# HKPolyU-UAV/bluerov2

Measured on AMD Instinct MI355X. Metric: NMPC RTI solves/s (N=20, 12 states / 4 inputs), batch 4096 per GPU, higher is better.
Workload: dtype f64; 1 GPU; BASELINE.json configs[1]: batch=4096 independent BlueROV2 NMPC instances per GPU, N=20, Ts=0.05 s, circle reference window advancing one row per step, per-instance x0 noise (seed 1), nominal parameters, default options (qp_early_exit=1: exact equality-constrained shortcut when no bound is active); batch_per_gpu=4096, N=20, parallelism=single GPU

## Files before the change

bluerov2_amd/csrc/qp/fused.hpp:

```cpp
#pragma once

namespace brov {

constexpr int kFusedMaxN = 23;
template <int W, bool GRID, bool DF>
__device__ __forceinline__ bool rti_fused_step(const DevParams& P, int b, int lane, bool listed, size_t yoff) {
    extern __shared__ __attribute__((aligned(16))) double smem[];
    const int N = P.N;
    double* ba_s = smem;
    double* bv_s = ba_s + (size_t)N * kBaStage;
    double* kt_s = bv_s + (size_t)N * NX;
    double* kff_s = kt_s + (size_t)N * kKtStage;
    double* vh_s = kff_s + (size_t)N * 4;
    double* dx_s = vh_s + (size_t)N * 4;
    double* q_s = dx_s + (size_t)(N + 1) * NX;
    double* r_s = q_s + (size_t)(N + 1) * NX;
    double* const_s = r_s + (size_t)N * 4;
    if (lane == 0) { const_s[0] = 0.0; const_s[1] = 1.0; }
    LaneCst lc;
    if constexpr (W == 1) lc = load_lane_cst(P.cst, lane);
    double part = 0.0;
    bool nanp = false;
    lin_phase<W == 1, GRID>(P, b, 0, N, lane, ba_s, bv_s, kt_s, q_s, r_s, part, nanp, true, yoff);
    __syncthreads();
    if (P.dump_lin) copy_out_linearisation(P, b, 0, N, lane, ba_s, bv_s);
    std::conditional_t<GRID, InstGrid, Inst> I;
    setup_inst(P, I, b, lane, W == 1 ? &lc : nullptr, yoff);
    const bool listed_u = __builtin_amdgcn_readfirstlane((int)listed) != 0;
    I.ckpt = (N >= 8 && P.partial_refactor && listed_u) ? (N + 3) >> 2 : 0;
    I.lds_ba = (const lds_f64*)ba_s;
    I.lds_bv = (const lds_f64*)bv_s;
    I.lds_kt = (lds_f64*)kt_s;
    I.lds_q = (const lds_f64*)q_s;
    I.lds_r = (const lds_f64*)r_s;
    I.kff = kff_s;
    I.vhat = vh_s;
    I.dxb = dx_s;
    I.lds_kff = (lds_f64*)kff_s;
    I.lds_vhat = (lds_f64*)vh_s;
    I.lds_dxb = (lds_f64*)dx_s;
    I.lds_zero = (lds_f64*)const_s;
    I.lds_tr = (lds_f64*)const_s + 2;
    {
        const int rg = I.rg, cl = I.cl;
        const int zero = (int)(const_s - ba_s), one = zero + 1, kt0 = (int)(kt_s - ba_s);
        for (int r = 0; r < 3; r++) I.ba_off[r] = cl >= 3 ? (rg + 4 * r) * kBaStride + cl - 3 : ((r == 0 && rg == cl) ? one : zero);
        I.ba_str = cl >= 3 ? kBaStage : 0;
        for (int r = 0; r < 4; r++) {
            const int c = rg + 4 * r;
            I.bat_off[r] = cl >= NX ? zero : (c >= 3 ? cl * kBaStride + c - 3 : (c == cl ? one : zero));
        }
        I.bat_str = cl >= NX ? 0 : kBaStage;
        I.bat_str0 = (cl < NX && rg == 3) ? kBaStage : 0;
        for (int r = 0; r < 3; r++) I.kt_off[r] = cl < 4 ? kt0 + (rg + 4 * r) * 4 + cl : zero;
        I.kt_str = cl < 4 ? kKtStage : 0;
    }
    qp_body<W, std::conditional_t<GRID, InstGrid, Inst>, DF>(P, I, b, part, nanp);
    return I.ran_loop;
}
__device__ __forceinline__ void plant_step_wave(const DevParams& P, int b, int lane, int tk) {
    double x[NX], u[NU], k[NX], xs[NX], acc[NX];
    double* x0 = P.x0_rw + (size_t)b * NX;
#pragma unroll
    for (int j = 0; j < NX; j++) x[j] = x0[j];
#pragma unroll
    for (int j = 0; j < NU; j++) u[j] = P.res[b].u0[j];
    const ModelPar m = make_par(P.plant_pp + (size_t)b * NP);
    Wrench w = make_wrench(u);
    if (P.plant_rp) { w.k3 = P.plant_rp[(size_t)b * P.plant_rp_stride]; w.k4 = P.plant_rp[(size_t)b * P.plant_rp_stride + 1]; }
    const double h = P.plant_dt / P.plant_substeps;
    StagePoint sp;
    for (int s = 0; s < P.plant_substeps; s++) {
        model_f(x, w, m, NoWorldWrench{}, k, sp);
#pragma unroll
        for (int j = 0; j < NX; j++) { acc[j] = x[j] + (h / 6.0) * k[j]; xs[j] = x[j] + 0.5 * h * k[j]; }
        model_f(xs, w, m, NoWorldWrench{}, k, sp);
#pragma unroll
        for (int j = 0; j < NX; j++) { acc[j] += (h / 3.0) * k[j]; xs[j] = x[j] + 0.5 * h * k[j]; }
        model_f(xs, w, m, NoWorldWrench{}, k, sp);
#pragma unroll
        for (int j = 0; j < NX; j++) { acc[j] += (h / 3.0) * k[j]; xs[j] = x[j] + h * k[j]; }
        model_f(xs, w, m, NoWorldWrench{}, k, sp);
#pragma unroll
        for (int j = 0; j < NX; j++) x[j] = acc[j] + (h / 6.0) * k[j];
    }
    if (lane == 0) {
#pragma unroll
        for (int j = 0; j < NX; j++) x0[j] = x[j];
        if (P.plant_xlog) {
#pragma unroll
            for (int j = 0; j < NX; j++) P.plant_xlog[((size_t)tk * P.B + b) * NX + j] = x[j];
        }
        if (P.plant_ulog) {
#pragma unroll
            for (int j = 0; j < NU; j++) P.plant_ulog[((size_t)tk * P.B + b) * NU + j] = u[j];
        }
    }
}

template <int W, bool GRID = false, bool DF = false, bool MULTI = false>
__device__ __forceinline__ void rti_fused_body(const DevParams& P) {
    const int b = __builtin_amdgcn_readfirstlane(sched_map(P, blockIdx.x));
    const int lane = threadIdx.x;
    bool listed = sched_listed(P, b);
    if (blockIdx.x == 0) sched_zero_next(P, lane);
    DBG_STAMP(0);
    if constexpr (!MULTI) {
        (void)rti_fused_step<W, GRID, DF>(P, b, lane, listed, 0);
    } else {
#pragma clang loop unroll(disable)
        for (int tk = 0; tk < P.ticks; tk++) {
            int bq = b, lq = lane;
            asm volatile("s_mov_b32 %0, %0" : "+s"(bq));
            asm volatile("v_mov_b32 %0, %0" : "+v"(lq));
            listed = rti_fused_step<W, GRID, DF>(P, bq, lq, listed, (size_t)tk * (size_t)P.tick_yref);
            if (P.tick_status && lq == 0) P.tick_status[(size_t)tk * P.B + bq] = P.res[bq].status;
            __syncthreads();
            wave_fence();
            if (P.plant_pp) {
                plant_step_wave(P, bq, lq, tk);
                __syncthreads();
                wave_fence();
            }
        }
    }
}

}
```

bluerov2_amd/csrc/qp/qp_body.hpp:

```cpp
#pragma once

namespace brov {

#define DBG_STAMP(slot) do { if (P.dbg && lane == 0) {                                                                          \
        P.dbg[(size_t)b * 8 + (slot)] = __builtin_readcyclecounter();                                                           \
        if ((slot) == 0) P.dbg[(size_t)P.B * 8 + (size_t)b * 8 + 7] = __builtin_amdgcn_s_memrealtime();                        \
        if ((slot) == 0) P.dbg[(size_t)P.B * 8 + (size_t)b * 8 + 5] = ((unsigned long long)__builtin_amdgcn_s_getreg(63508) << 32) | __builtin_amdgcn_s_getreg(63492); \
        if ((slot) == 6) P.dbg[(size_t)P.B * 8 + (size_t)b * 8 + 6] = __builtin_amdgcn_s_memrealtime(); } } while (0)
#ifdef BROV_DBG_IPM
#define IPM_T(k) do { const unsigned long long t_ = __builtin_readcyclecounter(); ipm_t[k] += t_ - ipm_last; ipm_last = t_; } while (0)
#else
#define IPM_T(k) do { } while (0)
#endif

#ifdef BROV_DBG_LIN
#define LIN_T(k) do { __builtin_amdgcn_sched_barrier(0); lin_t[k] = __builtin_readcyclecounter(); __builtin_amdgcn_sched_barrier(0); } while (0)
#else
#define LIN_T(k) do { } while (0)
#endif

template <int LDS, class IT = Inst, bool DF = false, bool LONGV = false>
__device__ __forceinline__ void qp_body(const DevParams& P, IT& I, int b, double lin_part, bool lin_nan, Win* W = nullptr,
                                        bool pre_ok = true, bool pre_illc = false) {
    constexpr bool EL = (LDS == 1 || LDS == 2);
    const double* __restrict__ cst = P.cst;
    const int lane = I.lane, N = I.NT, nv = I.nv;
    DBG_STAMP(1);
    const int rg = I.rg;

    double* x_it = P.x + (size_t)b * (N + 1) * 12;
    double* u_it = P.u + (size_t)b * N * 4;
    double* pi_it = P.pi + (size_t)b * N * 12;
    double* lam_it = P.lam + (size_t)b * N * 8;
    double* V = I.ipm + (size_t)IPM_V * nv;
    double* TL = I.ipm + (size_t)IPM_TL * nv;
    double* TU = I.ipm + (size_t)IPM_TU * nv;
    double* LL = I.ipm + (size_t)IPM_LL * nv;
    double* LU = I.ipm + (size_t)IPM_LU * nv;
    double* GAM = I.ipm + (size_t)IPM_GAM * nv;
    double* RT = I.ipm + (size_t)IPM_RT * nv;
    double* DVA = I.ipm + (size_t)IPM_DVA * nv;
    double* ACT = I.ipm + (size_t)IPM_ACT * nv;
    const double* GRAD = EL ? (const double*)I.kff : (const double*)DVA;
    auto rd_vhat = [&](int j) -> double { if constexpr (EL) return I.lds_vhat[j]; else return I.vhat[j]; };
    auto wr_vhat = [&](int j, double v) { if constexpr (EL) I.lds_vhat[j] = v; else I.vhat[j] = v; };
    auto rd_dxb = [&](int j) -> double { if constexpr (EL) return I.lds_dxb[j]; else return I.dxb[j]; };
    auto rd_grad = [&](int j) -> double { if constexpr (EL) return I.lds_kff[j]; else return GRAD[j]; };

    double x0v[3], xiv[3];
    {
        const double* x0 = P.x0 + (size_t)b * 12;
#pragma unroll
        for (int r = 0; r < 3; r++) { x0v[r] = x0[rg + 4 * r]; xiv[r] = I.x[rg + 4 * r]; }
    }

    double ureg[2] = {0.0, 0.0};
    if constexpr (EL) {
#pragma unroll
        for (int t = 0; t < 2; t++)
            if (lane + 64 * t < nv) ureg[t] = I.u[lane + 64 * t];
    }
    int status = 0, iters = 0;
    double mu = 0.0, rho = 0.0;
    bool early = false, polished = false, use_vhat = false;
    int sched_p = -1;
    bool ok = pre_ok;
    constexpr bool PART = EL || LDS >= 3;
    bool illc0 = pre_illc;
    bool split0 = false;
    if constexpr (EL) split0 = I.ckpt > 0;
    if constexpr (EL) { if (split0) {
        BwdState S;
        wave_fence();
        bwd_init<true, LDS>(I, S);
#pragma clang loop unroll(disable)
        for (int ph = 0; ph < 2; ph++) {
            if (ph == 1) {
                if (I.ckpt == 0) break;
                double* ck = I.Kt;
#pragma unroll
                for (int r = 0; r < 3; r++) { ck[r * 64 + lane] = S.P[r]; ck[192 + r * 64 + lane] = S.pv[r]; }
            }
            bwd_chunk<true, LDS, false, true>(I, S, ph == 0 ? N : I.ckpt, ph == 0 ? I.ckpt : 0);
        }
        ok = S.ok;
        illc0 = S.illc;
    } }
    if constexpr (LDS < 3) { if (!split0) ok = riccati_backward<true, LDS, false, true>(I, &illc0); }
    d4 d0;
    double kkt = 0.0;
    {
#pragma unroll
        for (int r = 0; r < 3; r++) {
            d0[r] = x0v[r] - xiv[r];
            kkt_upd(kkt, d0[r]);
        }
        d0[3] = 0.0;
        double part = lin_part;
        bool nanp = lin_nan;
        if (kkt != kkt) nanp = true;
        kkt = wave_max(fmax(part, (kkt != kkt) ? 0.0 : kkt));
        if (__ballot(nanp) != 0ull) kkt = __builtin_nan("");
    }
    constexpr bool ROB = LDS != 2;
    bool robust = false, robust_ok = false;
    if constexpr (ROB) {
        robust_ok = kkt <= P.robust_kkt_max || P.robust_pivot == 3;
        if ((__ballot(illc0) != 0ull && P.robust_pivot && robust_ok) || P.robust_pivot == 2) {
            robust = true;
            I.ckpt = 0;
            ok = sw_backward<true, LDS, true, true>(I, W);
        }
    }
    DBG_STAMP(2);
    const double lbc = EL ? cst[32 + (lane & 3)] : 0.0, ubc = EL ? cst[36 + (lane & 3)] : 0.0;
    if (__ballot(!ok) != 0ull) {
        status = BROV_STATUS_QP_FAILURE;
    } else {
        sw_forward<LDS>(I, W, d0, cst);
        DBG_STAMP(3);
        bool feas = true;
        if constexpr (LDS >= 3) {
            feas = W->feas;
        } else if constexpr (EL) {
#pragma unroll
            for (int t = 0; t < 2; t++) {
                const int j = lane + 64 * t;
                if (j < nv) {
                    const double vj = rd_vhat(j), lb = lbc - ureg[t], ub = ubc - ureg[t];
                    if (!(vj >= lb && vj <= ub)) feas = false;
                }
            }
        } else {
            for (int j = lane; j < nv; j += 64) {
                const int m = j & 3;
                const double vj = rd_vhat(j), lb = cst[32 + m] - I.u[j], ub = cst[36 + m] - I.u[j];
                if (!(vj >= lb && vj <= ub)) feas = false;
            }
        }
        const bool allfeas = (__ballot(!feas) == 0ull);
        if (allfeas && P.early_exit) {
            early = true;
        } else {
#ifdef BROV_DBG_IPM
            unsigned long long ipm_t[8] = {0, 0, 0, 0, 0, 0, 0, 0}, ipm_last = __builtin_readcyclecounter();
#endif
            constexpr bool CACHE = (LDS >= 3) && !LONGV;
            constexpr int kIpmT = EL ? 2 : ((LDS == 0 || LONGV) ? 16 : 8);
            using Vec = IpmVec<EL ? 1 : (CACHE ? 2 : 0), kIpmT>;
            Vec vV{{}, V}, vTL{{}, TL}, vTU{{}, TU}, vLL{{}, LL}, vLU{{}, LU}, vDVA{{}, DVA},
                vDLL{{}, GAM}, vDLU{{}, RT},
                vACT{{}, ACT};
#define IPM_FOR(t, j) _Pragma("unroll") for (int t = 0; t < kIpmT; t++) if (const unsigned j = (unsigned)lane + 64u * t; j < (unsigned)nv)
#define IPM_PRE(arr, expr)                                                                     \
            double arr[CACHE ? kIpmT : 1];                                                         \
            if constexpr (CACHE) {                                                                 \
                _Pragma("unroll") for (int t = 0; t < kIpmT; t++) {                                \
                    const unsigned j = ((unsigned)lane + 64u * t < (unsigned)nv) ? (unsigned)lane + 64u * t : 0u; \
                    arr[t] = (expr);                                                               \
                }                                                                                  \
            }
            auto set_act = [&](int t, int j, double v) __attribute__((always_inline)) { if constexpr (CACHE) ACT[j] = v; else vACT.set(t, j, v); };
#define GROUP_LANE int lane_g_ = I.lane; asm volatile("v_mov_b32 %0, %0" : "+v"(lane_g_)); const int lane = lane_g_
            const int mI = lane & 3;
            double lbI = cst[32 + mI], ubI = cst[36 + mI], wuI = cst[12 + mI];
            asm volatile("" : "+v"(lbI), "+v"(ubI), "+v"(wuI));
            const double rdI = P.Ts * wuI;
            auto rd_el = [&](unsigned j) __attribute__((always_inline)) -> double {
                if constexpr (LDS == 0) return I.wst ? I.wst[(size_t)(j >> 2) * 16 + 12 + mI] : rdI;
                else if constexpr (IT::kGrid) return I.wst[(size_t)(j >> 2) * 16 + 12 + mI];
                else return rdI;
            };
            {
                GROUP_LANE;
// ... 261 lines not shown
                    amax = wave_min(amax);
                    {
                        const double a = amax < 1.0 ? amax : 1.0;
                        alpha = (IPM_FTB * amax >= 1.0) ? 1.0 : a * ((1.0 - a) * IPM_FTBLO + a * IPM_FTB);
                    }
                    IPM_FOR(t, j) {
                        const double dv = (CACHE ? vh[CACHE ? t : 0] : rd_vhat(j)) - vV.get(t, j);
                        const double vj = vV.get(t, j) + alpha * dv;
                        const double tl = vTL.get(t, j) + alpha * dv, tu = vTU.get(t, j) - alpha * dv;
                        double dll, dlu;
                        if constexpr (CACHE) {
                            const double l0 = vLL.get(t, j), u0_ = vLU.get(t, j), t0_ = vTL.get(t, j), t1_ = vTU.get(t, j), dva = vDVA.get(t, j);
                            const double dlla = -l0 - l0 / t0_ * dva, dlua = -u0_ + u0_ / t1_ * dva;
                            dll = (smu - dlla * dva) / t0_ - l0 - l0 / t0_ * dv;
                            dlu = (smu + dlua * dva) / t1_ - u0_ + u0_ / t1_ * dv;
                        } else {
                            dll = vDLL.get(t, j); dlu = vDLU.get(t, j);
                        }
                        const double ll = vLL.get(t, j) + alpha * dll, lu = vLU.get(t, j) + alpha * dlu;
                        vV.set(t, j, vj); vTL.set(t, j, tl); vTU.set(t, j, tu); vLL.set(t, j, ll); vLU.set(t, j, lu);
                        if (!(vj == vj)) bad = true;
                        s2 += ll * tl + lu * tu;
                        const double rde = rd_el(j), al = ll / rde, au = lu / rde;
                        unres = fmax(unres, fmax(fmin(tl, al), fmin(tu, au)));
                        set_act(t, j, al > tl ? -1.0 : (au > tu ? 1.0 : 0.0));
                    }
                    vV.flush(lane, nv); vTL.flush(lane, nv); vTU.flush(lane, nv); vLL.flush(lane, nv); vLU.flush(lane, nv);
                    }
                if (__ballot(bad) != 0ull) { status = BROV_STATUS_NAN; break; }
                rho *= (1.0 - alpha);
                mu = wave_sum(s2) * inv2nv;
                IPM_T(1);
                unres = wave_max(unres);
                if (unres <= P.tol_mu && rho <= P.tol_stat) converged = true;
                if (converged || (mu <= POL_MU_GATE * mu_gate && alpha >= POL_ALPHA_GATE)) { round_k = 0; round_cap = POL_LOOP; nchg_prev = nv + 1; }
            }
            if (converged && status == BROV_STATUS_MAXITER) status = BROV_STATUS_SUCCESS;
#ifdef BROV_DBG_IPM
            if (P.dbg && lane == 0) {
                ipm_t[6] = iters;
                for (int k = 0; k < 7; k++) P.dbg[(size_t)P.B * 8 + (size_t)b * 8 + k] = ipm_t[k];
            }
#endif
            use_vhat = polished || !ipm_on;
            if (!polished) {
                if (ipm_on) {
                    if constexpr (EL) { IPM_FOR(t, j) wr_vhat(j, vV.get(t, j)); }
                } else if (status == BROV_STATUS_MAXITER) {
                    GROUP_LANE;
                    IPM_PRE(up, I.u[j]);
                    IPM_PRE(vh, I.vhat[j]);
                    IPM_FOR(t, j) {
                        const double uj = EL ? ureg[t & 1] : (CACHE ? up[CACHE ? t : 0] : I.u[j]);
                        double vj = CACHE ? vh[CACHE ? t : 0] : rd_vhat(j);
                        vj = fmin(fmax(vj, lbI - uj), ubI - uj);
                        if constexpr (EL) wr_vhat(j, vj); else I.vhat[j] = vj;
                    }
                }
            }
#undef IPM_FOR
#undef IPM_PRE
#undef GROUP_LANE
        }
    }

    bool emitted = false;
    auto emit_record = [&](double cost_lane, double u0_lane, bool have_u0) __attribute__((always_inline)) {
        const double cs = wave_sum(cost_lane);
        if (lane == 0) {
            brov_result* r = P.res + b;
            r->cost = cs;
            r->kkt = kkt;
            r->status = status;
            r->qp_iter = early ? 0 : iters;
        }
        double u0r = u0_lane;
        if (!have_u0 && lane < 4) {
            u0r = P.res[b].u0[lane];
            u0r = (u0r == u0r) ? u0r : 0.0;
            u0r = fmin(fmax(u0r, cst[32 + lane]), cst[36 + lane]);
            P.res[b].u0[lane] = u0r;
        }
        const double a0 = readlane_f64(u0r, 0), a1 = readlane_f64(u0r, 1), a2 = readlane_f64(u0r, 2), a3 = readlane_f64(u0r, 3);
        const double s0 = (lane == 0 || lane == 1) ? -a0 : a0;
        const double s1 = (lane == 0 || lane == 2) ? a1 : -a1;
        const double s3 = (lane == 0 || lane == 3) ? a3 : -a3;
        const double th = ((lane < 4) ? (s0 + s1) + s3 : -a2) / kRotor;
        if (lane < 6) P.res[b].thrust[lane] = th;
        if (P.mail) {
            brov_result* m = P.mail + b;
            if (lane < 4) m->u0[lane] = u0r;
            if (lane < 6) m->thrust[lane] = th;
            if (lane == 0) { m->cost = cs; m->kkt = kkt; m->status = status; m->qp_iter = early ? 0 : iters; }
            if (P.mail_flag) {
                __threadfence_system();
                if (lane == 0) __hip_atomic_store(P.mail_flag + b, P.mail_seq, __ATOMIC_RELEASE, __HIP_MEMORY_SCOPE_SYSTEM);
            }
        }
        emitted = true;
    };

    constexpr int UX = EL ? 5 : 4, UU = EL ? 2 : 4;
    const double* vfin = (early || EL || use_vhat) ? I.vhat : V;
    const int nxe = (N + 1) * 12;
    double cost = 0.0;
    bool wrote_u0 = false;
    double u0v = 0.0;
    if (status == BROV_STATUS_SUCCESS || status == BROV_STATUS_MAXITER) {
        if (!early && !polished) {
            sw_rollout<LDS>(I, W, d0, vfin);
        }
        DBG_STAMP(4);
        if constexpr (LDS >= 3) {
            if (W->nan) {
                status = BROV_STATUS_NAN;
            } else {
                win_adjoint_commit<LDS == 4>(P, I, *W, b, vfin, early, cost, u0v, P.mail != nullptr && P.mail_early != 0,
                                             [&](double cost_lane, double u0_lane) __attribute__((always_inline)) { emit_record(cost_lane, u0_lane, true); });
                wrote_u0 = true;
            }
            DBG_STAMP(5);
        } else {
        double xpre[UX], ypre[UX], urpre[UU];
        double wxpre[LDS == 1 ? UX : 1], wupre[LDS == 1 ? UU : 1];
        if constexpr (EL) {
#pragma unroll
            for (int t = 0; t < UX; t++) {
                const int j = lane + 64 * t;
                const int jj = j < nxe ? j : 0;
                const int i = div12(jj), c = jj - i * 12;
                xpre[t] = x_it[jj];
                ypre[t] = I.yref[(size_t)i * 16 + c];
                if constexpr (LDS == 1) wxpre[t] = cst[(i == N) ? 16 + c : c];
            }
#pragma unroll
            for (int t = 0; t < UU; t++) {
                const int j = lane + 64 * t;
                const int jj = j < nv ? j : 0;
                urpre[t] = I.yref[(size_t)(jj >> 2) * 16 + 12 + (jj & 3)];
                if constexpr (LDS == 1) wupre[t] = cst[12 + (jj & 3)];
            }
        }
        auto copy_pi = [&]() __attribute__((always_inline)) {
            double pv5[5];
#pragma unroll
            for (int t = 0; t < 5; t++) pv5[t] = I.lds_kt[lane + 64 * t < N * 12 ? lane + 64 * t : 0];
#pragma unroll
            for (int t = 0; t < 5; t++) asm volatile("" : "+v"(pv5[t]));
#pragma unroll
            for (int t = 0; t < 5; t++)
                if (lane + 64 * t < N * 12) pi_it[lane + 64 * t] = pv5[t];
        };
        const bool late = DF && EL && early && P.mail != nullptr;
        if (!(EL && polished) && !late) sw_adjoint<true, LDS>(I, W, vfin, DVA, pi_it);
        DBG_STAMP(5);
        bool nanv = false;
        double vvp[EL ? UU : 1], djp[EL ? UX : 1];
        if constexpr (EL) {
#pragma unroll
            for (int t = 0; t < UU; t++) vvp[t] = rd_vhat(lane + 64 * t < nv ? lane + 64 * t : 0);
#pragma unroll
            for (int t = 0; t < UX; t++) djp[t] = rd_dxb(lane + 64 * t < nxe ? lane + 64 * t : 0);
#pragma unroll
            for (int t = 0; t < UU; t++) nanv = nanv || !(vvp[t] == vvp[t]);
#pragma unroll
            for (int t = 0; t < UX; t++) nanv = nanv || !(djp[t] == djp[t]);
        } else {
            for (int j = lane; j < nv; j += 64) {
                const double vj = vfin[j];
                if (!(vj == vj)) nanv = true;
            }
            for (int j = lane; j < nxe; j += 64) {
                const double dj = rd_dxb(j);
                if (!(dj == dj)) nanv = true;
            }
        }
        if (__ballot(nanv) != 0ull) {
            status = BROV_STATUS_NAN;
        } else {
            for (int j0 = lane; j0 < nv; j0 += 64 * UU) {
                double uo[UU], vv[UU], gg[UU], ur[UU];
#pragma unroll
                for (int t = 0; t < UU; t++) {
                    const int j = j0 + 64 * t;
                    const bool in = j < nv;
                    const int jj = in ? j : 0;
                    uo[t] = (EL && j0 == lane && t < 2) ? ureg[t] : u_it[jj];
                    vv[t] = EL ? ((j0 == lane) ? vvp[EL ? t : 0] : rd_vhat(jj)) : vfin[jj];
                    gg[t] = early ? 0.0 : rd_grad(jj);
                    ur[t] = (EL && j0 == lane) ? urpre[t] : I.yref[(size_t)(jj >> 2) * 16 + 12 + (jj & 3)];
                }
#pragma unroll
                for (int t = 0; t < UU; t++) {
                    const int j = j0 + 64 * t;
                    if (j < nv) {
                        const int i = j >> 2, m = j & 3;
                        lam_it[i * 8 + m] = gg[t] > 0 ? gg[t] : 0.0;
                        lam_it[i * 8 + 4 + m] = gg[t] < 0 ? -gg[t] : 0.0;
                        const double un = uo[t] + vv[t];
                        u_it[j] = un;
                        if (j < 4) { P.res[b].u0[j] = un; u0v = un; }
                        const double e = un - ur[t];
                        const double wgt = (LDS == 1 && j0 == lane) ? wupre[LDS == 1 ? t : 0] : cst[12 + m];
                        const double sw = (IT::kGrid || (LDS == 0 && I.wst)) ? I.wst[(size_t)i * 16 + 12 + m] : P.Ts * wgt;
                        cost += 0.5 * sw * e * e;
                    }
                }
            }
            wrote_u0 = true;
            if constexpr (EL) {
                if (!late) copy_pi();
            }
            for (int j0 = lane; j0 < nxe; j0 += 64 * UX) {
                double xo[UX], dj[UX], yr[UX];
#pragma unroll
                for (int t = 0; t < UX; t++) {
                    const int j = j0 + 64 * t;
                    const int jj = j < nxe ? j : 0;
                    const int i = div12(jj), c = jj - i * 12;
                    xo[t] = (EL && j0 == lane) ? xpre[t] : x_it[jj];
                    dj[t] = (EL && j0 == lane) ? djp[EL ? t : 0] : rd_dxb(jj);
                    yr[t] = (EL && j0 == lane) ? ypre[t] : I.yref[(size_t)i * 16 + c];
                }
#pragma unroll
                for (int t = 0; t < UX; t++) {
                    const int j = j0 + 64 * t;
                    if (j < nxe) {
                        const int i = div12(j), c = j - i * 12;
                        const double xn = xo[t] + dj[t];
                        x_it[j] = xn;
                        const double e = xn - yr[t];
                        const double wgt = (LDS == 1 && j0 == lane) ? wxpre[LDS == 1 ? t : 0] : cst[(i == N) ? 16 + c : c];
                        const double sw = (IT::kGrid || (LDS == 0 && I.wst)) ? I.wst[(size_t)i * 16 + c] : ((i == N) ? wgt : P.Ts * wgt);
                        cost += 0.5 * sw * e * e;
                    }
                }
            }
        }
        if constexpr (DF && EL) {
            if (late && status == BROV_STATUS_SUCCESS) {
                emit_record(cost, u0v, wrote_u0);
                sw_adjoint<true, LDS>(I, W, vfin, DVA, pi_it);
                copy_pi();
            } else if (late) {
            }
        }
        }
    }
    if (status != BROV_STATUS_SUCCESS && status != BROV_STATUS_MAXITER) {
        const double* x0 = P.x0 + (size_t)b * 12;
        const double xl = x0[lane < 12 ? lane : 0];
        const bool restart = P.on_failure == BROV_ON_FAILURE_RESTART && __ballot(!(fabs(xl) < 1e300)) == 0ull;
        for (int j = lane; j < nv; j += 64) {
            const int i = j >> 2, m = j & 3;
            const double e = u_it[j] - I.yref[(size_t)i * 16 + 12 + m];
            cost += 0.5 * ((IT::kGrid || (LDS == 0 && I.wst)) ? I.wst[(size_t)i * 16 + 12 + m] : P.Ts * cst[12 + m]) * e * e;
            if (restart) { u_it[j] = 0.0; lam_it[i * 8 + m] = 0.0; lam_it[i * 8 + 4 + m] = 0.0; }
        }
        for (int j = lane; j < nxe; j += 64) {
            const int i = j / 12, c = j - i * 12;
            const double e = x_it[j] - I.yref[(size_t)i * 16 + c];
            cost += 0.5 * ((IT::kGrid || (LDS == 0 && I.wst)) ? I.wst[(size_t)i * 16 + c] : ((i == N) ? cst[16 + c] : P.Ts * cst[c])) * e * e;
            if (restart) { x_it[j] = x0[c]; if (i < N) pi_it[j] = 0.0; }
        }
    }
    if (!emitted) emit_record(cost, u0v, wrote_u0);
#ifdef BROV_SCHED_TICKET_LATE
    if (sched_p == -2) sched_p = sched_ticket(P, b);
#endif
    sched_note(P, b, sched_p);
    I.ran_loop = !early;
    DBG_STAMP(6);
}


struct LaneCst { double Wr[4], Wer[3], lbm, ubm, Wq, Weq, Wuq; };
__device__ __forceinline__ LaneCst load_lane_cst(const double* __restrict__ cst, int lane) {
    const int rg = lane >> 4;
    LaneCst c;
#pragma unroll
    for (int r = 0; r < 4; r++) c.Wr[r] = cst[rg + 4 * r];
#pragma unroll
    for (int r = 0; r < 3; r++) c.Wer[r] = cst[16 + rg + 4 * r];
    c.lbm = cst[32 + rg];
    c.ubm = cst[36 + rg];
    const int cq = (lane >> 2) < NX ? (lane >> 2) : NX - 1;
    c.Wq = cst[cq];
    c.Weq = cst[16 + cq];
    c.Wuq = cst[12 + ((lane >> 2) & 3)];
    return c;
}
__device__ __forceinline__ void setup_inst(const DevParams& P, Inst& I, int b, int lane, const LaneCst* pre = nullptr, size_t yoff = 0) {
    const int N = P.N, nv = 4 * N;
    const double* __restrict__ cst = P.cst;
    I.lane = lane; I.rg = lane >> 4; I.cl = lane & 15; I.N = N; I.nv = nv;
    I.i0 = 0; I.NT = N; I.ckpt = 0;
    I.x = P.x + (size_t)b * (N + 1) * 12;
    I.u = P.u + (size_t)b * N * 4;
    I.yref = P.yref + yoff + (size_t)b * P.yref_stride;
    I.BA = P.BA + (size_t)b * N * 192;
    I.bvec = P.bvec + (size_t)b * N * 12;
    I.Ks = P.Ks + (size_t)b * N * 64;
    I.Kt = P.Kt + (size_t)b * N * 192;
    I.Mt = P.Mt + (size_t)b * N * 64;
    I.Pb = P.Pb + (size_t)b * N * 12;
    I.kff = P.kff + (size_t)b * N * 4;
    I.vhat = P.vhat + (size_t)b * N * 4;
    I.ipm = P.ipm + (size_t)b * IPM_NARR * nv;
    I.dxb = P.dxb + (size_t)b * (N + 1) * 12;
    I.Ts = P.Ts;
    I.wst = P.wst;
    I.lds_ba = nullptr;
    I.lds_bv = nullptr;
    I.lds_kt = nullptr;
    I.lds_q = nullptr;
    I.lds_r = nullptr;
    I.lds_kff = nullptr;
    I.lds_vhat = nullptr;
    I.lds_dxb = nullptr;
    I.lds_zero = nullptr;
    I.lds_tr = nullptr;
    const LaneCst c = pre ? *pre : load_lane_cst(cst, lane);
#pragma unroll
    for (int r = 0; r < 4; r++) I.Wr[r] = c.Wr[r];
#pragma unroll
    for (int r = 0; r < 3; r++) I.Wer[r] = c.Wer[r];
    I.lbm = c.lbm;
    I.ubm = c.ubm;
    I.Wq = c.Wq; I.Weq = c.Weq; I.Wuq = c.Wuq;
}

}
```

bluerov2_amd/csrc/qp/sweeps.hpp:

```cpp
#pragma once

namespace brov {

template <int LDS> constexpr int kLdsDist = LDS == 2 ? 1 : 2;

struct BwdIn {
    d4 ba;
    d4 bv;
    double xv[3], yv[3];
    double rtv, gm;
    double ks, mt;
};

struct Ba1Off { int off[3], str; };
template <bool FACTOR, int LDS, bool STEP0 = false, class IT = Inst>
__device__ __forceinline__ BwdIn load_bwd(const IT& I, int i, const double* gam, const double* rt, const Ba1Off* b1 = nullptr) {
    BwdIn s;
    s.ba = get_ba<LDS>(I, i);
    const int ig = I.i0 + i;
    if constexpr (FACTOR && LDS != 0) {
        if (b1) {
            const lds_f64* t = I.lds_ba + lmul(i, b1->str);
            s.bv = d4{t[b1->off[0]], t[b1->off[1]], t[b1->off[2]], 0.0};
        } else {
// ... 551 lines not shown
        const bool rowx = k < NX;
        const double e0 = (q == 0 && k == 0) ? 1.0 : 0.0, e1 = (q == 0 && k == 1) ? 1.0 : 0.0, e2 = (q == 0 && k == 2) ? 1.0 : 0.0;
        lds_f64* xpark = rowx ? I.lds_dxb + NX + k : I.lds_tr + (I.lane & 15);
        const int xstr = rowx ? NX : 0;
        const int ka = rowx ? k : NX - 1, c0 = 4 * q - 3;
        const int oa = ka * kBaStride + (c0 > 0 ? c0 : 0), oa3 = ka * kBaStride + c0 + 3, ob = ka;
        const lds_f64* zr0 = q < 3 ? I.lds_dxb + 4 * q : I.lds_vhat;
        const int zstr = q < 3 ? NX : 4;
        double z0 = zr0[0], z1 = zr0[1], z2 = zr0[2], z3 = zr0[3];
        pipelined<kLdsDist<LDS>, RollV>(N, [&](int kk) { return load_roll_v(I, oa, oa3, ob, kk); }, [&](int i, const RollV& in) {
            const double a0 = q == 0 ? e0 : in.a[0], a1 = q == 0 ? e1 : in.a[1], a2 = q == 0 ? e2 : in.a[2];
            double pa = a0 * z0;
            pa = fma(a1, z1, pa); pa = fma(a2, z2, pa); pa = fma(in.a[3], z3, pa);
            const double xn = quad_sum(pa) + in.bk;
            xpark[lmul(i, xstr)] = rowx ? xn : 0.0;
            const lds_f64* zr = zr0 + lmul(i + 1 < N ? i + 1 : i, zstr);
            z0 = zr[0]; z1 = zr[1]; z2 = zr[2]; z3 = zr[3];
        });
        const lds_f64* xl = I.lds_dxb + N * NX + rg;
        xx = d4{xl[0], xl[4], xl[8], 0.0};
    } else {
        pipelined<3, RollIn>(N, [&](int k) { return load_roll<LDS>(I, k, varr); }, [&](int i, const RollIn& in) {
            d4 z = {xx[0], xx[1], xx[2], in.v};
            xx = tn<4>(in.bat, z, in.bb);
            xx[3] = 0.0;
            store_vec12(I.dxb + (size_t)(i + 1) * 12, xx, rg, cl);
        });
    }
}
template <int LDS>
__device__ void rollout(const Inst& I, const d4& d0, const double* varr) {
    wave_fence();
    d4 xx = d0;
    roll_chunk<LDS>(I, xx, varr);
    wave_fence();
}

struct AdjIn { d4 ba; double dx[3], xn[3], yn[3]; double v, u, ur; };
template <int LDS>
__device__ __forceinline__ AdjIn load_adj(const Inst& I, int i, const double* varr) {
    AdjIn s;
    s.ba = get_ba<LDS>(I, i);
    const double* dxn = I.dxb + (size_t)(i + 1) * 12;
    if constexpr (LDS) s.v = I.lds_vhat[i * 4 + I.rg]; else s.v = varr[i * 4 + I.rg];
    if constexpr (LDS) {
        const lds_f64* dxl = I.lds_dxb + (i + 1) * 12;
#pragma unroll
        for (int r = 0; r < 3; r++) { s.dx[r] = dxl[I.rg + 4 * r]; s.xn[r] = I.lds_q[(i + 1) * 12 + I.rg + 4 * r]; s.yn[r] = 0.0; }
        s.u = I.lds_r[i * 4 + I.rg];
        s.ur = 0.0;
    } else {
        const double* xn = I.x + (size_t)(i + 1) * 12;
        const double* yn = I.yref + (size_t)(i + 1) * 16;
#pragma unroll
        for (int r = 0; r < 3; r++) { s.dx[r] = dxn[I.rg + 4 * r]; s.xn[r] = xn[I.rg + 4 * r]; s.yn[r] = yn[I.rg + 4 * r]; }
        s.u = I.u[i * 4 + I.rg];
        s.ur = I.yref[(size_t)i * 16 + 12 + I.rg];
    }
    return s;
}
struct AdjV { double m[4], dxc, qc, vm, rm, wq, wr; };
template <class IT = Inst>
__device__ __forceinline__ AdjV load_adj_v(const IT& I, int om, int ox, int ou, int i) {
    AdjV s;
    const lds_f64* col = I.lds_ba + i * kBaStage + om;
#pragma unroll
    for (int t = 0; t < 4; t++) s.m[t] = col[t * kBaStride];
    s.dxc = I.lds_dxb[(i + 1) * NX + ox];
    s.qc = I.lds_q[(i + 1) * NX + ox];
    s.vm = I.lds_vhat[i * 4 + ou];
    s.rm = I.lds_r[i * 4 + ou];
    s.wq = 0.0; s.wr = 0.0;
    if constexpr (IT::kGrid) {
        s.wq = I.wst[(size_t)(I.i0 + i + 1) * 16 + ox];
        s.wr = I.wst[(size_t)(I.i0 + i) * 16 + 12 + ou];
    }
    return s;
}
template <bool COMMIT, int LDS, class IT = Inst>
__device__ __forceinline__ void adj_chunk(const IT& I, d4& atpi, const double* varr, double* garr, double* pi_out) {
    const int rg = I.rg, cl = I.cl, N = I.N;
    if constexpr (LDS) {
        const int c = I.lane >> 2, q = I.lane & 3;
        const bool rowx = c < NX, colx = q < 3;
        const int q3 = colx ? q : 2;
        const double e0 = (colx && 4 * q == c) ? 1.0 : 0.0, e1 = (colx && 4 * q + 1 == c) ? 1.0 : 0.0, e2 = (colx && 4 * q + 2 == c) ? 1.0 : 0.0,
                     e3 = (colx && 4 * q + 3 == c) ? 1.0 : 0.0;
        const bool ecol = c < 3;
        const int om = (4 * q3) * kBaStride + (c >= 3 ? c - 3 : 0), ox = rowx ? c : NX - 1, ou = c & 3;
        store_vec12_lds(I.lds_tr, atpi, rg, cl);
        double gq = I.lds_tr[rowx ? c : 0];
        lds_f64* ppark = rowx ? I.lds_kt + c : I.lds_tr + (I.lane & 15);
        const int pstr = rowx ? NX : 0;
        lds_f64* gpark = rowx ? I.lds_tr + (I.lane & 15) : I.lds_kff + (c - NX);
        const int gstr = rowx ? 0 : 4;
        const double rd = I.Ts * I.Wuq;
        lds_f64* pp = ppark + lmul(N - 1, pstr);
        lds_f64* gp = gpark + lmul(N - 1, gstr);
        pipelined<kLdsDist<LDS>, AdjV>(N, [&](int kk) { return load_adj_v(I, om, ox, ou, N - 1 - kk); }, [&](int kk, const AdjV& in) {
            const int i = N - 1 - kk;
            const double qd = IT::kGrid ? in.wq : ((I.i0 + i + 1 == I.NT) ? I.Weq : I.Ts * I.Wq);
            const double pic = fma(qd, in.dxc, in.qc + gq);
            *pp = pic; pp -= pstr;
            const lds_f64* pr = I.lds_kt + i * NX + 4 * q3;
            const double p0 = pr[0], p1 = pr[1], p2 = pr[2], p3 = pr[3];
            __builtin_amdgcn_sched_barrier(0);
            const double m0 = ecol ? e0 : in.m[0], m1 = ecol ? e1 : in.m[1], m2 = ecol ? e2 : in.m[2], m3 = ecol ? e3 : in.m[3];
            double acc = m0 * p0;
            acc = fma(m1, p1, acc); acc = fma(m2, p2, acc); acc = fma(m3, p3, acc);
            acc = colx ? acc : 0.0;
            const double G = quad_sum(acc);
            *gp = fma(IT::kGrid ? in.wr : rd, in.vm, in.rm + G); gp -= gstr;
            gq = G;
        });
        lds_f64* tpark = rowx ? I.lds_tr + c : I.lds_tr + 16;
        *tpark = gq;
        const lds_f64* tl = I.lds_tr + rg;
        atpi = d4{tl[0], tl[4], tl[8], 0.0};
        return;
    }
    const d4 z4 = {0, 0, 0, 0};
    auto stage = [&](int i, const AdjIn& in) __attribute__((always_inline)) {
        d4 pi;
        double wq[3], wr;
        if (I.wst) {
            const double* ws = I.wst + (size_t)(i + 1) * 16 + rg;
            wq[0] = ws[0]; wq[1] = ws[4]; wq[2] = ws[8];
            wr = I.wst[(size_t)i * 16 + 12 + rg];
        } else {
#pragma unroll
            for (int r = 0; r < 3; r++) wq[r] = (I.i0 + i + 1 == I.NT) ? I.Wer[r] : I.Ts * I.Wr[r];
            wr = I.Ts * I.Wr[3];
        }
#pragma unroll
        for (int r = 0; r < 3; r++) pi[r] = wq[r] * (in.dx[r] + in.xn[r] - in.yn[r]) + atpi[r];
        pi[3] = 0.0;
        if (COMMIT) store_vec12(pi_out + (size_t)i * 12, pi, rg, cl);
        d4 G = tn<3>(in.ba, pi, z4);
        const double rd = wr;
        if (cl == 0) garr[i * 4 + rg] = rd * in.v + rd * (in.u - in.ur) + G[3];
        atpi = G;
    };
    pipelined<3, AdjIn>(N, [&](int k) { return load_adj<LDS>(I, N - 1 - k, varr); },
                        [&](int k, const AdjIn& in) { stage(N - 1 - k, in); });
}
template <bool COMMIT, int LDS, class IT = Inst>
__device__ void adjoint(const IT& I, const double* varr, double* garr, double* pi_out) {
    wave_fence();
    d4 atpi = {0, 0, 0, 0};
    adj_chunk<COMMIT, LDS>(I, atpi, varr, garr, pi_out);
    wave_fence();
}

}
```

Measured before the change: 5.725 million solves/s.

## Interleave early-exit solution writeback into a specialized adjoint sweep

Adds a specialized path for the one-wave fused kernel on the uniform grid when the equality-constrained early exit is taken. A new software-pipelined adjoint sweep computes the multipliers from LDS data, and the per-lane u/x writeback, lambda zeroing and cost accumulation are spliced into its peeled tail iterations. The goal is to hide global stores and arithmetic behind the serial adjoint recursion instead of running them afterwards. This adds template specialization and more code complexity, and duplicates logic that must stay consistent with the generic tail.

Result: no change. 5.753 million solves/s, median of 6 (+0.5%).

```diff
diff --git a/bluerov2_amd/csrc/qp/fused.hpp b/bluerov2_amd/csrc/qp/fused.hpp
--- a/bluerov2_amd/csrc/qp/fused.hpp
+++ b/bluerov2_amd/csrc/qp/fused.hpp
@@ -3,7 +3,7 @@
 namespace brov {
 
 constexpr int kFusedMaxN = 23;
-template <int W, bool GRID, bool DF>
+template <int W, bool GRID, bool DF, bool ET = false>
 __device__ __forceinline__ bool rti_fused_step(const DevParams& P, int b, int lane, bool listed, size_t yoff) {
     extern __shared__ __attribute__((aligned(16))) double smem[];
     const int N = P.N;
@@ -55,7 +55,7 @@
         for (int r = 0; r < 3; r++) I.kt_off[r] = cl < 4 ? kt0 + (rg + 4 * r) * 4 + cl : zero;
         I.kt_str = cl < 4 ? kKtStage : 0;
     }
-    qp_body<W, std::conditional_t<GRID, InstGrid, Inst>, DF>(P, I, b, part, nanp);
+    qp_body<W, std::conditional_t<GRID, InstGrid, Inst>, DF, false, ET>(P, I, b, part, nanp);
     return I.ran_loop;
 }
 __device__ __forceinline__ void plant_step_wave(const DevParams& P, int b, int lane, int tk) {
@@ -106,7 +106,7 @@
     if (blockIdx.x == 0) sched_zero_next(P, lane);
     DBG_STAMP(0);
     if constexpr (!MULTI) {
-        (void)rti_fused_step<W, GRID, DF>(P, b, lane, listed, 0);
+        (void)rti_fused_step<W, GRID, DF, W == 1 && !GRID && !DF>(P, b, lane, listed, 0);
     } else {
 #pragma clang loop unroll(disable)
         for (int tk = 0; tk < P.ticks; tk++) {
diff --git a/bluerov2_amd/csrc/qp/qp_body.hpp b/bluerov2_amd/csrc/qp/qp_body.hpp
--- a/bluerov2_amd/csrc/qp/qp_body.hpp
+++ b/bluerov2_amd/csrc/qp/qp_body.hpp
@@ -19,7 +19,7 @@
 #define LIN_T(k) do { } while (0)
 #endif
 
-template <int LDS, class IT = Inst, bool DF = false, bool LONGV = false>
+template <int LDS, class IT = Inst, bool DF = false, bool LONGV = false, bool ET = false>
 __device__ __forceinline__ void qp_body(const DevParams& P, IT& I, int b, double lin_part, bool lin_nan, Win* W = nullptr,
                                         bool pre_ok = true, bool pre_illc = false) {
     constexpr bool EL = (LDS == 1 || LDS == 2);
@@ -587,6 +587,61 @@
                 if (lane + 64 * t < N * 12) pi_it[lane + 64 * t] = pv5[t];
         };
         const bool late = DF && EL && early && P.mail != nullptr;
+        bool et_tail = false;
+        if constexpr (ET) {
+            static_assert(LDS == 1 && !IT::kGrid && !DF, "the one-wave fused kernel on the uniform grid");
+            if (early) {
+                et_tail = true;
+                double vvp[UU], djp[UX];
+                bool nanv = false;
+#pragma unroll
+                for (int t = 0; t < UU; t++) vvp[t] = rd_vhat(lane + 64 * t < nv ? lane + 64 * t : 0);
+#pragma unroll
+                for (int t = 0; t < UX; t++) djp[t] = rd_dxb(lane + 64 * t < nxe ? lane + 64 * t : 0);
+#pragma unroll
+                for (int t = 0; t < UU; t++) nanv = nanv || !(vvp[t] == vvp[t]);
+#pragma unroll
+                for (int t = 0; t < UX; t++) nanv = nanv || !(djp[t] == djp[t]);
+                if (__ballot(nanv) != 0ull) {
+                    status = BROV_STATUS_NAN;
+                } else {
+                    const double Ts = P.Ts;
+                    adjoint_early<UU + UX>(I, [&](auto sc) __attribute__((always_inline)) {
+                        constexpr int sl = decltype(sc)::value;
+                        if constexpr (sl < UU) {
+                            constexpr int t = sl;
+                            const int j = lane + 64 * t;
+                            if (j < nv) {
+                                const int i = j >> 2, m = j & 3;
+                                lam_it[i * 8 + m] = 0.0;
+                                lam_it[i * 8 + 4 + m] = 0.0;
+                                const double un = ureg[t] + vvp[t];
+                                u_it[j] = un;
+                                if (j < 4) { P.res[b].u0[j] = un; u0v = un; }
+                                const double e = un - urpre[t];
+                                const double sw = Ts * wupre[t];
+                                cost += 0.5 * sw * e * e;
+                            }
+                        } else {
+                            constexpr int t = sl - UU;
+                            const int j = lane + 64 * t;
+                            if (j < nxe) {
+                                const int i = div12(j);
+                                const double xn = xpre[t] + djp[t];
+                                x_it[j] = xn;
+                                const double e = xn - ypre[t];
+                                const double sw = (i == N) ? wxpre[t] : Ts * wxpre[t];
+                                cost += 0.5 * sw * e * e;
+                            }
+                        }
+                    });
+                    wrote_u0 = true;
+                    copy_pi();
+                }
+                DBG_STAMP(5);
+            }
+        }
+        if (!et_tail) {
         if (!(EL && polished) && !late) sw_adjoint<true, LDS>(I, W, vfin, DVA, pi_it);
         DBG_STAMP(5);
         bool nanv = false;
@@ -671,6 +726,7 @@
                     }
                 }
             }
+        }
         }
         if constexpr (DF && EL) {
             if (late && status == BROV_STATUS_SUCCESS) {
diff --git a/bluerov2_amd/csrc/qp/sweeps.hpp b/bluerov2_amd/csrc/qp/sweeps.hpp
--- a/bluerov2_amd/csrc/qp/sweeps.hpp
+++ b/bluerov2_amd/csrc/qp/sweeps.hpp
@@ -727,4 +727,72 @@
     wave_fence();
 }
 
-}
+struct AdjEV { double m[4], dxc, qc; };
+template <class F, int... Ks>
+__device__ __forceinline__ void for_const(std::integer_sequence<int, Ks...>, F f) { (f(std::integral_constant<int, Ks>{}), ...); }
+template <int NSL, class Slice>
+__device__ __forceinline__ void adjoint_early(const Inst& I, Slice slice) {
+    constexpr int D = kLdsDist<1>, S = D + 1, PEEL = NSL + S - 1;
+    wave_fence();
+    const int N = I.N;
+    const int c = I.lane >> 2, q = I.lane & 3;
+    const bool rowx = c < NX, colx = q < 3;
+    const int q3 = colx ? q : 2;
+    const double e0 = (colx && 4 * q == c) ? 1.0 : 0.0, e1 = (colx && 4 * q + 1 == c) ? 1.0 : 0.0, e2 = (colx && 4 * q + 2 == c) ? 1.0 : 0.0,
+                 e3 = (colx && 4 * q + 3 == c) ? 1.0 : 0.0;
+    const bool ecol = c < 3;
+    const int om = (4 * q3) * kBaStride + (c >= 3 ? c - 3 : 0), ox = rowx ? c : NX - 1;
+    double gq = 0.0;
+    lds_f64* ppark = rowx ? I.lds_kt + c : I.lds_tr + (I.lane & 15);
+    const int pstr = rowx ? NX : 0;
+    lds_f64* pp = ppark + lmul(N - 1, pstr);
+    auto load = [&](int kk) __attribute__((always_inline)) {
+        const int i = N - 1 - (kk < N ? kk : N - 1);
+        AdjEV s;
+        const lds_f64* col = I.lds_ba + i * kBaStage + om;
+#pragma unroll
+        for (int t = 0; t < 4; t++) s.m[t] = col[t * kBaStride];
+        s.dxc = I.lds_dxb[(i + 1) * NX + ox];
+        s.qc = I.lds_q[(i + 1) * NX + ox];
+        return s;
+    };
+    auto stage = [&](int kk, const AdjEV& in, auto sl) __attribute__((always_inline)) {
+        const int i = N - 1 - kk;
+        const double qd = (I.i0 + i + 1 == I.NT) ? I.Weq : I.Ts * I.Wq;
+        const double pic = fma(qd, in.dxc, in.qc + gq);
+        *pp = pic; pp -= pstr;
+        const lds_f64* pr = I.lds_kt + i * NX + 4 * q3;
+        const double p0 = pr[0], p1 = pr[1], p2 = pr[2], p3 = pr[3];
+        if constexpr (decltype(sl)::value >= 0) {
+            __builtin_amdgcn_sched_barrier(0);
+            slice(sl);
+        }
+        __builtin_amdgcn_sched_barrier(0);
+        const double m0 = ecol ? e0 : in.m[0], m1 = ecol ? e1 : in.m[1], m2 = ecol ? e2 : in.m[2], m3 = ecol ? e3 : in.m[3];
+        double acc = m0 * p0;
+        acc = fma(m1, p1, acc); acc = fma(m2, p2, acc); acc = fma(m3, p3, acc);
+        acc = colx ? acc : 0.0;
+        gq = quad_sum(acc);
+    };
+    AdjEV slot[S];
+#pragma unroll
+    for (int d = 0; d < D; d++) slot[d] = load(d);
+    const int M = N > NSL ? (N - NSL) / S * S : 0;
+    for (int k = 0; k < M; k += S) {
+#pragma unroll
+        for (int d = 0; d < S; d++) {
+            slot[(d + D) % S] = load(k + d + D);
+            stage(k + d, slot[d], std::integral_constant<int, -1>{});
+        }
+    }
+    for_const(std::make_integer_sequence<int, PEEL>{}, [&](auto pc) __attribute__((always_inline)) {
+        constexpr int p = decltype(pc)::value;
+        slot[(p + D) % S] = load(M + p + D);
+        if (M + p < N) stage(M + p, slot[p % S], std::integral_constant<int, (p < NSL ? p : -1)>{});
+    });
+    if (N < NSL)
+        for_const(std::make_integer_sequence<int, NSL>{}, [&](auto sc) __attribute__((always_inline)) { if (N <= decltype(sc)::value) slice(sc); });
+    wave_fence();
+}
+
+}
```
